# daviszhen/plan

Hardware: AMD Instinct MI355X
Metric: rows/sec through hash-agg (Q1) (higher is better)
Workload: dtype int64; 1 GPU; TPC-H Q1 fused filter+hash-aggregate over lineitem, 59986052 rows on rank 0, 59986052 in total (SF10 per GPU), table resident in HBM; rows_per_gpu=59986052, kernel_family=lowcard_chain, groups=4, rows_aggregated=58682142, parallelism=single GPU, rccl_ranks=1

## Files before the change

### include/planhip.h

```cpp
#ifndef PLANHIP_H
#define PLANHIP_H

#include <stdint.h>

#ifdef __cplusplus
extern "C" {
#endif

#define PH_OK 0
#define PH_EINVAL (-1)
#define PH_EHIP (-2)
#define PH_EUNSUPPORTED (-3)
#define PH_EOVERFLOW (-4)
#define PH_ECAPACITY (-5)
#define PH_ECONSTRAINT (-6)

typedef struct ph_ctx ph_ctx;

const char *ph_last_error(void);
const char *ph_version(void);

int ph_ctx_create(int device, ph_ctx **out);
int ph_ctx_set_stream(ph_ctx *ctx, void *hip_stream);
int ph_ctx_sync(ph_ctx *ctx);
// ... 153 lines not shown

#define PH_STAT_ASCENDING 1
#define PH_STAT_STRICT 2
#define PH_STAT_DECLARED_UNIQUE 4
int ph_table_col_stats(const ph_table *t, int32_t c, int32_t *flags);
int32_t ph_table_col_run_len(const ph_table *t, int32_t c);
int ph_table_col_narrow(const ph_table *t, int32_t c, int32_t *width, int64_t *base);
int64_t ph_table_narrow_bytes(const ph_table *t);
int ph_table_declare_unique(ph_table *t, int32_t ncols, const int32_t *cols);
int ph_table_colocate(ph_table *t, int32_t ncols, const int32_t *cols);
int32_t ph_table_colocated(const ph_table *t, int32_t ncols, const int32_t *cols);
int ph_table_set_colocate_budget(ph_table *t, int64_t bytes);
int64_t ph_table_colocate_bytes(const ph_table *t);
int ph_table_pack_scan_group(ph_table *t, int32_t ncols, const int32_t *cols);
int64_t ph_table_scan_group_bytes(const ph_table *t);
int ph_pack_scan_layout(int32_t nfields, const int32_t *widths, int32_t *shifts);
int32_t ph_pack_scan_bits(uint64_t span);
void ph_table_free(ph_table *t);

int ph_dev_alloc(ph_ctx *ctx, int64_t bytes, void **dev);
int ph_dev_free(ph_ctx *ctx, void *dev);
int ph_dev_free_many(ph_ctx *ctx, void *const *devs, int64_t n);
int ph_dev_upload(ph_ctx *ctx, void *dev, const void *host, int64_t bytes);
int ph_dev_download(ph_ctx *ctx, void *host, const void *dev, int64_t bytes);
int ph_dev_memset(ph_ctx *ctx, void *dev, int value, int64_t bytes);

typedef enum { PH_EQ = 1, PH_NE, PH_LT, PH_LE, PH_GT, PH_GE, PH_LIKE, PH_NOTLIKE } ph_cmp;

typedef struct {
    int32_t type;
// ... 347 lines not shown
```

### plan_amd/csrc/common.h

```cpp
#pragma once

#include <hip/hip_runtime.h>

#include <atomic>
#include <cstdarg>
#include <cstdint>
#include <cstdio>
#include <cstdlib>
#include <cstring>
#include <deque>
#include <map>
#include <mutex>
#include <string>
#include <vector>

#include "dispatch.h"
#include "planhip.h"

namespace ph {

void set_error(const char *fmt, ...);

#define PH_HIP(call)                                                                     \
    do {                                                                                 \
// ... 132 lines not shown
        void *data = nullptr;
        int64_t bytes = 0;
        void *ready = nullptr;
        hipStream_t built_on = nullptr;
        bool complete = false;
    };
    std::deque<colgroup> groups;
    std::map<std::vector<int>, int> sparse_gathers;
    bool replicated = false;
    int64_t colocate_budget = 4ll << 30;
    int64_t colocate_bytes = 0;
    struct scangroup {
        std::vector<int> cols;
        int32_t shift[6] = {0, 0, 0, 0, 0, 0}, width[6] = {0, 0, 0, 0, 0, 0};
        int32_t nk1 = 0, nslots = 0;
        void *data = nullptr;
        int64_t bytes = 0;
        void *ready = nullptr;
        hipStream_t built_on = nullptr;
        bool complete = false;
    };
    std::deque<scangroup> scan_groups;
    std::map<std::vector<int>, int64_t> lean_rows;
    int64_t scan_group_bytes = 0;
};

namespace ph {
template <auto Kernel>
int raise_lds(ph_ctx *ctx, int bytes) {
    static std::atomic<int> raised[64];
// ... 2 lines not shown
    int current = -1;
    PH_HIP(hipGetDevice(&current));
    if (current != ctx->device) {
        ph::set_error("raise_lds: the current device is %d, the context's is %d", current, ctx->device);
        return PH_EINVAL;
    }
    PH_HIP(hipFuncSetAttribute(reinterpret_cast<const void *>(Kernel), hipFuncAttributeMaxDynamicSharedMemorySize, bytes));
    r.store(bytes, std::memory_order_release);
    return PH_OK;
}

void register_table(ph_table *t);
void unregister_table(ph_table *t);
bool lookup_table_col(const void *data, ph_table **t, int *col);
int colocated_group_for(ph_ctx *ctx, ph_table *t, const std::vector<int> &tc, bool may_build, bool explicit_request, ph_table::colgroup *out);
int scan_group_for(ph_ctx *ctx, ph_table *t, const int32_t cols[7], int64_t rows, bool explicit_request, ph_table::scangroup *out);
bool scan_pack_enabled();
int table_finish_column(ph_ctx *ctx, ph_table::column &d, int64_t nrows, int64_t padded, const void *dict_blob, int64_t dict_bytes);
bool narrow_enabled();
}

constexpr int64_t PH_ROW_PAD = 8192;
```

### plan_amd/csrc/ctx.hip

```cpp
#include <algorithm>

#include "common.h"
#include "scan_kernels.h"

namespace ph {

static thread_local char g_err[512] = "";

void set_error(const char *fmt, ...) {
    va_list ap;
    va_start(ap, fmt);
    vsnprintf(g_err, sizeof g_err, fmt, ap);
    va_end(ap);
}

}

extern "C" const char *ph_last_error(void) { return ph::g_err; }
extern "C" const char *ph_version(void) { return "planhip 0.1 (gfx950)"; }

int ph_ctx::ensure_scratch(int64_t bytes) {
    if (bytes <= scratch_bytes) return PH_OK;
    if (scratch) {
        PH_HIP(hipStreamSynchronize(stream));
// ... 857 lines not shown
    int shift[ph::PACK_NFIELDS];
};
__global__ __launch_bounds__(256) void pack_scan_kernel(PackScanParams P, int64_t n, unsigned long long *__restrict__ out) {
    for (int64_t r = (int64_t)blockIdx.x * 256 + threadIdx.x; r < n; r += (int64_t)gridDim.x * 256) {
        unsigned long long word = (unsigned long long)((unsigned)P.k0[r] * (unsigned)P.nk1 + (unsigned)P.k1[r]) << P.shift[ph::PF_SLOT];
        for (int c = 0; c < 5; c++) {
            const unsigned long long code = P.w[c] == 1   ? ((const uint8_t *)P.src[c])[r]
                                            : P.w[c] == 2 ? ((const uint16_t *)P.src[c])[r]
                                                          : ((const uint32_t *)P.src[c])[r];
            word |= code << P.shift[c];
        }
        out[r] = word;
    }
}

namespace ph {
bool scan_pack_enabled() {
    static const bool on = !(getenv("PH_SCAN_PACK") && getenv("PH_SCAN_PACK")[0] == '0');
    return on;
}
}

static int64_t scan_pack_min_bytes() {
    if (const char *e = getenv("PH_SCAN_PACK_MIN_BYTES")) return atoll(e);
    return 256ll << 20;
}

static bool scan_group_shape(const ph_table *t, const int32_t cols[7], ph_table::scangroup *g, std::string *why) {
    auto no = [&](const std::string &s) { *why = s; return false; };
    if (!ph::narrow_enabled()) return no("the narrowed copies are switched off");
    for (int i = 0; i < 7; i++) {
        if (cols[i] < 0 || cols[i] >= (int32_t)t->cols.size()) return no("bad column " + std::to_string(cols[i]));
        for (int j = 0; j < i; j++) if (cols[j] == cols[i]) return no("column " + std::to_string(cols[i]) + " is named twice");
    }
    static const int want_w[5] = {2, 1, 4, 1, 1};
    int32_t width[ph::PACK_NFIELDS];
    for (int i = 0; i < 5; i++) {
        const ph_table::column &c = t->cols[(size_t)cols[i]];
        const bool i32 = c.type == PH_I32 || c.type == PH_DATE, i64 = c.type == PH_I64 || c.type == PH_DEC64;
        if (c.validity || !(i < 2 ? i32 : i64)) return no("column " + std::to_string(cols[i]) + " is NULL-able or not of its role's integer type");
// ... 7 lines not shown
        n[i] = c.dict.empty() ? (int)c.max + 1 : (int)c.dict.size();
        if (!c.has_range || c.min < 0 || c.max >= n[i]) return no("column " + std::to_string(cols[5 + i]) + " holds codes outside its dictionary");
    }
    if (n[0] * n[1] <= 0 || n[0] * n[1] > ph::LC_MAX_SLOTS) return no(std::to_string(n[0] * n[1]) + " group slots exceed " + std::to_string(ph::LC_MAX_SLOTS));
    g->nk1 = n[1];
    g->nslots = n[0] * n[1];
    width[ph::PF_SLOT] = ph::pack_bits((uint64_t)(g->nslots - 1));
    if (!ph::pack_layout(ph::PACK_NFIELDS, width, g->shift)) return no("the fields do not fit one 64-bit word without straddling its dwords");
    g->cols.assign(cols, cols + 7);
    std::copy(width, width + ph::PACK_NFIELDS, g->width);
    return true;
}

static int pack_scan_locked(ph_ctx *ctx, ph_table *t, ph_table::scangroup g, bool explicit_request) {
    const int64_t padded = ph::round_up(t->nrows > 0 ? t->nrows : 1, PH_ROW_PAD);
    g.bytes = padded * 8;
    if (!explicit_request && t->colocate_bytes + t->scan_group_bytes + g.bytes > t->colocate_budget) return PH_ECAPACITY;
    PH_HIP(hipSetDevice(ctx->device));
    PH_HIP(hipMalloc(&g.data, (size_t)g.bytes));
    hipEvent_t ev = nullptr;
    if (hipEventCreateWithFlags(&ev, hipEventDisableTiming) != hipSuccess) { (void)hipFree(g.data); ph::set_error("ph_table_pack_scan_group: hipEventCreate failed"); return PH_EHIP; }
    auto fail = [&]() { (void)hipEventDestroy(ev); (void)hipFree(g.data); ph::set_error("ph_table_pack_scan_group: launch failed"); return PH_EHIP; };
    if (hipMemsetAsync((char *)g.data + t->nrows * 8, 0, (size_t)((padded - t->nrows) * 8), ctx->stream) != hipSuccess) return fail();
    if (t->nrows > 0) {
        PackScanParams P{};
        for (int i = 0; i < 5; i++) { P.src[i] = t->cols[(size_t)g.cols[(size_t)i]].narrow; P.w[i] = t->cols[(size_t)g.cols[(size_t)i]].narrow_w; }
        P.k0 = (const uint8_t *)t->cols[(size_t)g.cols[5]].data;
        P.k1 = (const uint8_t *)t->cols[(size_t)g.cols[6]].data;
        P.nk1 = g.nk1;
        for (int f = 0; f < ph::PACK_NFIELDS; f++) P.shift[f] = g.shift[f];
        pack_scan_kernel<<<(int)std::min<int64_t>((t->nrows + 255) / 256, 256 * 16), 256, 0, ctx->stream>>>(P, t->nrows, (unsigned long long *)g.data);
        if (hipGetLastError() != hipSuccess) return fail();
    }
    if (hipEventRecord(ev, ctx->stream) != hipSuccess) return fail();
    g.ready = ev;
    g.built_on = ctx->stream;
    t->scan_group_bytes += g.bytes;
    t->scan_groups.push_back(g);
    return PH_OK;
}

int ph::scan_group_for(ph_ctx *ctx, ph_table *t, const int32_t cols[7], int64_t rows, bool explicit_request, ph_table::scangroup *out) {
    if (!explicit_request && !scan_pack_enabled()) return PH_EUNSUPPORTED;
    std::lock_guard<std::mutex> lock(t->mu);
    const std::vector<int> key(cols, cols + 7);
    auto find = [&]() -> ph_table::scangroup * {
        for (auto &g : t->scan_groups) if (g.cols == key) return &g;
        return nullptr;
    };
    ph_table::scangroup *g = find();
    if (!g) {
        if (explicit_request) {
            ph_table::scangroup shape;
            std::string why;
            if (!scan_group_shape(t, cols, &shape, &why)) { ph::set_error("ph_table_pack_scan_group: %s", why.c_str()); return PH_EUNSUPPORTED; }
            PH_CHECK(pack_scan_locked(ctx, t, shape, true));
        } else {
            int64_t &seen = t->lean_rows[key];
            if (seen < 0) return PH_EUNSUPPORTED;
            seen += rows;
            if (seen < 2 * t->nrows || t->nrows <= 0) return PH_EUNSUPPORTED;
            const int64_t padded = ph::round_up(t->nrows, PH_ROW_PAD);
            if (padded * 11 <= scan_pack_min_bytes()) { seen = 2 * t->nrows; return PH_EUNSUPPORTED; }
            ph_table::scangroup shape;
            std::string why;
            if (!scan_group_shape(t, cols, &shape, &why) || pack_scan_locked(ctx, t, shape, false) != PH_OK) {
                (void)hipGetLastError();
                seen = -1;
                return PH_EUNSUPPORTED;
            }
        }
        g = find();
        if (!g) return PH_EUNSUPPORTED;
    }
    if (!g->complete && g->built_on != ctx->stream) {
        const hipError_t q = hipEventQuery((hipEvent_t)g->ready);
        if (q == hipSuccess) g->complete = true;
        else if (q == hipErrorNotReady) PH_HIP(hipStreamWaitEvent(ctx->stream, (hipEvent_t)g->ready, 0));
        else { ph::set_error("packed scan group: %s", hipGetErrorString(q)); return PH_EHIP; }
    }
    *out = *g;
    return PH_OK;
}

extern "C" int ph_table_pack_scan_group(ph_table *t, int32_t ncols, const int32_t *cols) {
    PH_REQUIRE(t && t->ctx && cols && ncols == 7, "ph_table_pack_scan_group: seven columns (predicate, q, e, d, t and the two group columns)");
    ph_table::scangroup g;
    return ph::scan_group_for(t->ctx, t, cols, 0, true, &g);
}

extern "C" int64_t ph_table_scan_group_bytes(const ph_table *t) {
    if (!t) return -1;
    std::lock_guard<std::mutex> lock(const_cast<ph_table *>(t)->mu);
    return t->scan_group_bytes;
}

extern "C" int ph_pack_scan_layout(int32_t nfields, const int32_t *widths, int32_t *shifts) {
    PH_REQUIRE(widths && shifts, "ph_pack_scan_layout: bad arguments");
    if (!ph::pack_layout(nfields, widths, shifts)) { ph::set_error("ph_pack_scan_layout: the fields do not fit one 64-bit word without straddling its dwords"); return PH_EUNSUPPORTED; }
    return PH_OK;
}

extern "C" int32_t ph_pack_scan_bits(uint64_t span) { return ph::pack_bits(span); }
// ... 47 lines not shown
```

### plan_amd/csrc/pack_layout.h

```cpp
#pragma once
#include <cstdint>

namespace ph {

constexpr int PACK_NFIELDS = 6;
enum PackField { PF_P = 0, PF_Q, PF_E, PF_D, PF_T, PF_SLOT };

constexpr int pack_bits(uint64_t span) {
    int b = 1;
    while (b < 64 && (span >> b) != 0) b++;
    return b;
}

constexpr bool pack_layout(int n, const int32_t *width, int32_t *shift) {
    if (n < 1 || n > 64) return false;
    bool placed[64] = {};
    int used[2] = {0, 0};
    for (int i = 0; i < n; i++)
        if (width[i] < 1 || width[i] > 32) return false;
    for (int k = 0; k < n; k++) {
        int best = -1;
        for (int i = 0; i < n; i++)
            if (!placed[i] && (best < 0 || width[i] > width[best])) best = i;
        const int dw = used[0] + width[best] <= 32 ? 0 : used[1] + width[best] <= 32 ? 1 : -1;
// ... 5 lines not shown
    return true;
}

struct PackLayout {
    int32_t width[PACK_NFIELDS], shift[PACK_NFIELDS];
    bool ok;
};
constexpr PackLayout lineitem_pack_layout() {
    PackLayout L = {{12, 6, 24, 4, 4, 3}, {}, false};
    L.ok = pack_layout(PACK_NFIELDS, L.width, L.shift);
    return L;
}
constexpr PackLayout LCP_LINEITEM = lineitem_pack_layout();
static_assert(LCP_LINEITEM.ok, "lineitem's 53 bits fit one word");

inline bool is_lineitem_layout(const uint8_t *shift, const uint8_t *width) {
    for (int f = 0; f < PACK_NFIELDS; f++)
        if (shift[f] != LCP_LINEITEM.shift[f] || width[f] != LCP_LINEITEM.width[f]) return false;
    return true;
}

}
```

### plan_amd/csrc/scan_inst.h

```cpp
#pragma once
#include <algorithm>
#include <cstdint>

namespace ph {

enum ScanForm : int32_t { FORM_WIDE = 0, FORM_NARROW = 1, FORM_NARROW32 = 2 };

constexpr int LC_BINS_MAX_SLOTS = 6;
constexpr int LC_BINS_MAX_TILES = 1023;

struct ScanSwitches {
    bool nt = true, narrow_generic = false, pack_generic = false, lean = true, tail = true, hist = true;
    int unroll = 1, grid = 0;
};

enum FsInst { FSI_WIDE, FSI_NARROW_RT64, FSI_NARROW_RT32, FSI_NARROW_FIXED32 };
enum LcInst { LCI_WIDE, LCI_NARROW_RT64, LCI_NARROW_RT32, LCI_NARROW_FIXED32, LCI_LEAN, LCI_PACKED_RT, LCI_PACKED_FIXED, LCI_BINS };

inline FsInst narrow_inst(int32_t form, bool lineitem_widths, const ScanSwitches &s) {
    if (form == FORM_NARROW) return FSI_NARROW_RT64;
    return !s.nt || s.narrow_generic || !lineitem_widths ? FSI_NARROW_RT32 : FSI_NARROW_FIXED32;
}

struct FsFacts {
    int32_t form = FORM_WIDE;
    int32_t w[4] = {0, 0, 0, 0};
};
inline FsInst fs_choose(const FsFacts &f, const ScanSwitches &s) {
    if (f.form == FORM_WIDE) return FSI_WIDE;
    return narrow_inst(f.form, f.w[0] == 2 && f.w[1] == 1 && f.w[2] == 1 && f.w[3] == 4, s);
}
inline const char *fs_variant_name(FsInst i) {
    return i == FSI_WIDE ? "wide" : i == FSI_NARROW_RT64 ? "narrow64" : i == FSI_NARROW_RT32 ? "narrow_rt" : "narrow32";
}

struct LcFacts {
    int32_t form = FORM_WIDE;
    int32_t w[5] = {0, 0, 0, 0, 0};
    bool lean = false, group_bound = false, group_lineitem = false;
    int32_t nslots = 0;
    bool tiles_fit = true;
};
inline LcInst lc_choose(const LcFacts &f, const ScanSwitches &s) {
    if (f.group_bound) {
        const bool fixed = f.group_lineitem && !s.pack_generic;
        if (fixed && s.hist && f.nslots <= LC_BINS_MAX_SLOTS && f.tiles_fit) return LCI_BINS;
        return fixed ? LCI_PACKED_FIXED : LCI_PACKED_RT;
    }
    if (f.form == FORM_WIDE) return LCI_WIDE;
    const FsInst n = narrow_inst(f.form, f.w[0] == 2 && f.w[1] == 1 && f.w[2] == 4 && f.w[3] == 1 && f.w[4] == 1, s);
    return n == FSI_NARROW_RT64 ? LCI_NARROW_RT64 : n == FSI_NARROW_RT32 ? LCI_NARROW_RT32 : f.lean ? LCI_LEAN : LCI_NARROW_FIXED32;
}
inline bool lc_takes_lean(LcFacts f, const ScanSwitches &s) {
    f.group_bound = false;
    return lc_choose(f, s) == LCI_LEAN;
}
inline bool lc_takes_bins(LcInst i) { return i == LCI_BINS; }
inline const char *lc_variant_name(LcInst i) {
    return i == LCI_WIDE ? "wide" : i == LCI_NARROW_RT64 ? "narrow64" : i == LCI_NARROW_RT32 ? "narrow_rt" : i == LCI_NARROW_FIXED32 ? "narrow32"
         : i == LCI_LEAN ? "narrow32_lean" : "packed64";
}
inline const char *lc_row_body_name(LcInst i) { return lc_takes_bins(i) ? "bins" : "columns"; }

struct ScanGeometry {
    int64_t tile_rows, tiles;
    int grid;
    bool bins;
};
inline ScanGeometry scan_geometry(int64_t row_begin, int64_t rows, bool narrow, int max_grid, int grid_override, bool bins_eligible, int partials_cap) {
    ScanGeometry g;
    g.tile_rows = narrow ? 4096 : 1024;
    const int64_t span = rows > 0 && narrow ? rows + (row_begin & 15) : rows;
    g.tiles = (span + g.tile_rows - 1) / g.tile_rows;
    if (grid_override > 0) max_grid = std::min(grid_override, partials_cap);
    g.grid = (int)std::min<int64_t>(max_grid, std::max<int64_t>(g.tiles, 1));
    g.bins = bins_eligible;
    if (g.bins && (g.tiles + g.grid - 1) / g.grid > LC_BINS_MAX_TILES) {
        const int64_t need = (g.tiles + LC_BINS_MAX_TILES - 1) / LC_BINS_MAX_TILES;
        if (need <= partials_cap) g.grid = (int)need;
        else g.bins = false;
    }
    return g;
}

}
```

### plan_amd/csrc/scan_kernels.h

```cpp
#pragma once
#include "common.h"
#include "pack_layout.h"
#include "scan_inst.h"

namespace ph {

constexpr int LC_NACC = 6;
constexpr int LC_MAX_SLOTS = 12;
constexpr int SCAN_TAIL_MAX_ACC = 128;
struct ScanTail {
    unsigned *done;
    unsigned long long *out_lo;
    long long *out_hi;
    int32_t nacc, min_stride;
    unsigned long long *mbox;
    unsigned long long *flag;
    unsigned long long seq;
};

struct ForCol {
    const uint8_t *data;
    int64_t base;
    int32_t w;
};
// ... 20 lines not shown
    const uint8_t *k0, *k1;
    int32_t p_lo, p_hi;
    int32_t nk1;
    int32_t nslots;
    int64_t A1, B1, A2, B2;
    int64_t row_begin, row_end;
    long long *partials;
    ScanTail tail;
    int32_t form;
    ForCol np, nq, ne, nd, nt;
    uint32_t np_lo, np_hi;
    int32_t lean;
    int32_t A1c, B1c, A2c, B2c, e_base32;
    const uint8_t *pk;
    uint8_t pk_shift[PACK_NFIELDS], pk_width[PACK_NFIELDS];
    int32_t bins;
};

int launch_filter_sumprod(ph_ctx *ctx, const FilterSumProdParams &P, FsInst inst, const ScanSwitches &sw, int grid);
int launch_lowcard_chain(ph_ctx *ctx, const LowcardChainParams &P, LcInst inst, const ScanSwitches &sw, int grid);
int launch_merge_partials(ph_ctx *ctx, const long long *partials, int nblocks, int nacc,
                          int min_stride, unsigned long long *out_lo, long long *out_hi, const ScanTail *publish = nullptr);

int launch_merge_partials_ops(ph_ctx *ctx, const long long *partials, int nblocks, int nacc, int stride,
                              unsigned long long opmask, unsigned long long *out_lo, long long *out_hi, const ScanTail *publish = nullptr);

}
```

### plan_amd/csrc/scan_kernels.hip

```cpp

#include "common.h"
#include "scan_kernels.h"

namespace ph {


__device__ __forceinline__ long long wave_sum_i64(long long v) {
    for (int o = 32; o > 0; o >>= 1) v += __shfl_xor(v, o);
    return v;
}

struct alignas(16) i64x2 { long long x, y; };
struct alignas(16) i32x4 { int x, y, z, w; };

typedef long long v2i64 __attribute__((ext_vector_type(2)));
typedef int v4i32 __attribute__((ext_vector_type(4)));

template <bool NT> __device__ __forceinline__ i64x2 ld_i64x2(const int64_t *p) {
    if (NT) {
        v2i64 v = __builtin_nontemporal_load(reinterpret_cast<const v2i64 *>(p));
        return i64x2{v.x, v.y};
    }
    return *reinterpret_cast<const i64x2 *>(p);
}
// ... 809 lines not shown
    lds_char *c32 = (lds_char *)(cols + threadIdx.x);

    const int64_t tile_rows = 4096;
    const bool none = P.np_lo > P.np_hi;
    const unsigned sp = P.np_hi - P.np_lo;
    const int64_t rb = P.row_begin, re = none ? 0 : P.row_end;
    int64_t tile0 = (rb & ~(int64_t)15) + (int64_t)blockIdx.x * tile_rows;
    int64_t row = tile0 + (threadIdx.x >> 6) * (8 * LCP_GROUP) + (threadIdx.x & 63) * 2;
    const int64_t stride = (int64_t)gridDim.x * tile_rows;
#define LCH_BODY(M, T) lch_rows<M>(LCP_ARGS(T), P, row, rb, re, sp, b64, c32)
    PH_LEAN_TILE_LOOP(LCP_DECL, LCP_LOAD, LCH_BODY)
#undef LCH_BODY
    lch_fold(P, lds_acc, bins, cols, red, ns);
}

__device__ __forceinline__ void merge_finish(const ScanTail &T, int j, unsigned long long lo, long long hi, unsigned long long *out_lo, long long *out_hi) {
    const int lane = threadIdx.x;
    if (!T.done) {
        if (lane == 0) {
            out_lo[j] = lo;
            out_hi[j] = hi;
        }
        return;
    }
    unsigned ticket = 0;
    if (lane == 0) {
        __hip_atomic_store(out_lo + j, lo, __ATOMIC_RELAXED, __HIP_MEMORY_SCOPE_AGENT);
        __hip_atomic_store(out_hi + j, hi, __ATOMIC_RELAXED, __HIP_MEMORY_SCOPE_AGENT);
        __builtin_amdgcn_s_waitcnt(0);
        ticket = __hip_atomic_fetch_add(T.done, 1u, __ATOMIC_RELAXED, __HIP_MEMORY_SCOPE_AGENT);
// ... 104 lines not shown
    return PH_OK;
}

template <auto Kernel>
static int launch_lowcard_inst(ph_ctx *ctx, const LowcardChainParams &P, int grid, size_t lds) {
    PH_CHECK(raise_lds<Kernel>(ctx, 160 * 1024));
    Kernel<<<grid, 256, lds, ctx->stream>>>(P);
    PH_HIP(hipGetLastError());
    return PH_OK;
}

int launch_lowcard_chain(ph_ctx *ctx, const LowcardChainParams &P, LcInst inst, const ScanSwitches &sw, int grid) {
    const size_t lds = (size_t)P.nslots * (5 * 256 * sizeof(unsigned long long) + 2 * 256 * sizeof(unsigned));
    switch (inst) {
    case LCI_BINS: return launch_lowcard_inst<lowcard_chain_kernel_hist>(ctx, P, grid, lch_lds_bytes(P.nslots));
    case LCI_PACKED_FIXED: return launch_lowcard_inst<lowcard_chain_kernel_packed<true>>(ctx, P, grid, lds);
    case LCI_PACKED_RT: return launch_lowcard_inst<lowcard_chain_kernel_packed<false>>(ctx, P, grid, lds);
    case LCI_LEAN: return launch_lowcard_inst<lowcard_chain_kernel_lean>(ctx, P, grid, lds);
    case LCI_NARROW_FIXED32: return launch_lowcard_inst<lowcard_chain_kernel_for<true, true, 2, 1, 4, 1, 1>>(ctx, P, grid, lds);
    case LCI_NARROW_RT64: case LCI_NARROW_RT32:
        return dispatch_bool(sw.nt, [&](auto NT) { return dispatch_bool(inst == LCI_NARROW_RT32, [&](auto P32) {
            return launch_lowcard_inst<lowcard_chain_kernel_for<NT(), P32(), 0, 0, 0, 0, 0>>(ctx, P, grid, lds);
        }); });
    case LCI_WIDE:
        if (!sw.nt) return launch_lowcard_inst<lowcard_chain_kernel<false, 1>>(ctx, P, grid, lds);
        return dispatch_int<3, 2, 1>(sw.unroll, [&](auto U) { return launch_lowcard_inst<lowcard_chain_kernel<true, U()>>(ctx, P, grid, lds); });
    }
    return PH_EINVAL;
}

// ... 22 lines not shown
```

### plan_amd/csrc/scan_plan.hip

```cpp
#include <algorithm>
#include <cmath>

#include "common.h"
#include "scan_inst.h"
#include "scan_jit.h"
#include "scan_kernels.h"
#include "scan_lower.h"

namespace {

using ph::set_error;
using ph::Affine;
using ph::AggReq;
using ph::ColView;
using ph::Prod;
using ph::Range;

std::vector<ColView> col_views(const ph_table *t) {
    std::vector<ColView> v(t->cols.size());
    for (size_t i = 0; i < v.size(); i++) {
        const auto &c = t->cols[i];
        v[i] = ColView{c.type, c.scale, c.validity != nullptr, c.has_range, c.min, c.max, &c.dict};
    }
    return v;
// ... 90 lines not shown

extern "C" void ph_scan_plan_free(ph_scan_plan *p) {
    if (!p) return;
    if (p->partials) p->ctx->pool_release(p->partials);
    if (p->out_lo) p->ctx->pool_release(p->out_lo);
    if (p->g_agg) ph_agg_free(p->g_agg);
    delete p;
}


static ph::FsFacts fs_facts(const ph::FilterSumProdParams &P) { return ph::FsFacts{P.form, {P.np0.w, P.np2.w, P.nb.w, P.na.w}}; }

static ph::LcFacts lc_facts(const ph::LowcardChainParams &P, bool tiles_fit) {
    const bool group = P.pk != nullptr;
    return ph::LcFacts{P.form, {P.np.w, P.nq.w, P.ne.w, P.nd.w, P.nt.w}, P.lean != 0, group, group && ph::is_lineitem_layout(P.pk_shift, P.pk_width),
                       P.nslots, tiles_fit};
}

extern "C" const char *ph_scan_plan_kind(const ph_scan_plan *p) {
    if (!p) return "";
    return p->kind == PK_FILTER_SUMPROD ? "filter_sumprod" : p->kind == PK_LOWCARD_CHAIN ? "lowcard_chain" : p->kind == PK_JIT ? "jit" : "generic";
}

extern "C" int32_t ph_scan_plan_bytes_per_row(const ph_scan_plan *p) { return p ? p->bytes_per_row : 0; }

extern "C" const char *ph_scan_plan_variant(const ph_scan_plan *p) {
    if (!p) return "";
    if (p->kind == PK_FILTER_SUMPROD) return ph::fs_variant_name(ph::fs_choose(fs_facts(p->fs), process_switches()));
    if (p->kind == PK_LOWCARD_CHAIN) return ph::lc_variant_name(ph::lc_choose(lc_facts(p->lc, true), process_switches()));
    return ph_scan_plan_kind(p);
}

extern "C" const char *ph_scan_plan_row_body(const ph_scan_plan *p) {
    if (!p || p->kind != PK_LOWCARD_CHAIN || !(p->last_inst < 0 || p->last_inst == ph::LCI_BINS)) return "columns";
    ph::ScanSwitches sw = process_switches();
    sw.hist = hist_switch();
    return ph::lc_row_body_name(ph::lc_choose(lc_facts(p->lc, true), sw));
}


static int plan_filter_sumprod(ph_ctx *ctx, const ph_table *t, const std::vector<ColView> &cols, const std::vector<Range> &ranges,
                               const std::vector<AggReq> &reqs, ph_scan_plan *p) {
    p->kind = PK_FILTER_SUMPROD;
    int32_t a_col = -1, b_col = -1;
    for (size_t i = 0; i < reqs.size(); i++) {
        ph::AggMap m{reqs[i].kind, 1, 0};
        if (!reqs[i].star) {
            const Prod &pr = reqs[i].p;
            if (pr.f.size() != 2 || !pr.f[0].pure() || !pr.f[1].pure() || !is_i64(cols[pr.f[0].col]) || !is_i64(cols[pr.f[1].col])) {
// ... 467 lines not shown
    return sw;
}

static int bind_scan_group(ph_scan_plan *p, int64_t rows, const ph::ScanSwitches &sw) {
    if (p->lc.pk || !ph::lc_takes_lean(lc_facts(p->lc, true), sw)) return PH_OK;
    ph_table::scangroup g;
    const int rc = ph::scan_group_for(p->ctx, const_cast<ph_table *>(p->t), p->lc_cols, rows, false, &g);
    if (rc == PH_EUNSUPPORTED) return PH_OK;
    PH_CHECK(rc);
    if (g.nk1 != p->lc.nk1 || g.nslots != p->lc.nslots) return PH_OK;
    for (int f = 0; f < ph::PACK_NFIELDS; f++) {
        p->lc.pk_shift[f] = (uint8_t)g.shift[f];
        p->lc.pk_width[f] = (uint8_t)g.width[f];
    }
    p->lc.pk = (const uint8_t *)g.data;
    p->bytes_per_row = 8;
    return PH_OK;
}

static int arm_tail(ph_scan_plan *p, bool back_to_back, ph::ScanTail *tail) {
    *tail = ph::ScanTail{};
    if (!process_switches().tail || p->nacc > ph::SCAN_TAIL_MAX_ACC || (back_to_back && p->kind != PK_FILTER_SUMPROD)) return PH_OK;
    ph_ctx *ctx = p->ctx;
    if (!ctx->scan_done_dev) {
        PH_HIP(hipMalloc((void **)&ctx->scan_done_dev, 64));
        PH_HIP(hipMemsetAsync(ctx->scan_done_dev, 0, 64, ctx->stream));
    }
    tail->done = ctx->scan_done_dev;
    tail->out_lo = p->out_lo;
    tail->out_hi = p->out_hi;
    tail->nacc = p->nacc;
// ... 36 lines not shown
    PH_CHECK(ph::launch_lowcard_chain(p->ctx, P, inst, sw, grid));
    return ph::launch_merge_partials(p->ctx, p->partials, grid, p->nacc, ph::LC_NACC + 1, p->out_lo, p->out_hi, &tail);
}

extern "C" int ph_scan_plan_run(ph_scan_plan *p, int64_t row_begin, int64_t row_end) {
    PH_REQUIRE(p != nullptr, "ph_scan_plan_run: plan is NULL");
    const bool narrow = (p->kind == PK_FILTER_SUMPROD && p->fs.form != ph::FORM_WIDE) || (p->kind == PK_LOWCARD_CHAIN && p->lc.form != ph::FORM_WIDE);
    PH_REQUIRE(row_begin >= 0 && row_end >= row_begin && row_end <= p->t->nrows && (narrow || row_begin % 4 == 0),
               "ph_scan_plan_run: rows [%lld,%lld) invalid (begin must be a multiple of 4 unless the plan reads narrowed copies; table has %lld rows)",
               (long long)row_begin, (long long)row_end, (long long)p->t->nrows);
    if (p->kind == PK_GENERIC) return generic_run(p, row_begin, row_end);
    const ph::ScanSwitches sw = run_switches(p);
    const bool lowcard = p->kind == PK_LOWCARD_CHAIN;
    if (lowcard) PH_CHECK(bind_scan_group(p, row_end - row_begin, sw));
    const int64_t rows = p->never ? 0 : row_end - row_begin;
    const bool bins_eligible = lowcard && ph::lc_choose(lc_facts(p->lc, true), sw) == ph::LCI_BINS;
    const ph::ScanGeometry g = ph::scan_geometry(row_begin, rows, narrow, p->max_grid, sw.grid, bins_eligible, partials_cap(p));
    const ph::LcInst inst = lowcard ? ph::lc_choose(lc_facts(p->lc, g.bins), sw) : ph::LCI_WIDE;
    if (lowcard) p->last_inst = inst;
    const long double rows_per_block = (long double)((g.tiles + g.grid - 1) / g.grid) * (long double)g.tile_rows;
    if (p->row_bound * rows_per_block >= 4.0e18L) {
        set_error("decimal overflow proof failed: per-row bound %.3Lg x %.0Lf rows per workgroup", p->row_bound, rows_per_block);
        return PH_EOVERFLOW;
    }
    p->last_rows = rows;
    p->last_grid = g.grid;
    p->armed_seq = 0;
    const bool back_to_back = p->unfetched;
    p->unfetched = true;
    ph::ScanTail tail;
    PH_CHECK(arm_tail(p, back_to_back, &tail));
    if (p->kind == PK_FILTER_SUMPROD) return launch_filter_sumprod_plan(p, row_begin, rows, sw, g.grid, tail);
// ... 130 lines not shown
```

### plan_amd/hip.py

```python
import ctypes
import os

import numpy as np

_HERE = os.path.dirname(os.path.abspath(__file__))
_LIB = None

PH_JOIN_KEY_RANGE, PH_JOIN_FK_PROBES, PH_JOIN_KEYS_SORTED_UNIQUE, PH_JOIN_EXISTS_ONLY = 1, 2, 4, 8
PH_OK, PH_EINVAL, PH_EHIP, PH_EUNSUPPORTED, PH_EOVERFLOW, PH_ECAPACITY, PH_ECONSTRAINT = 0, -1, -2, -3, -4, -5, -6
PH_I32, PH_I64, PH_DATE, PH_DEC64, PH_CODE8, PH_F32, PH_F64, PH_STR = range(1, 9)
PH_EQ, PH_NE, PH_LT, PH_LE, PH_GT, PH_GE, PH_LIKE, PH_NOTLIKE = range(1, 9)
PH_X_COL, PH_X_CONST, PH_X_ADD, PH_X_SUB, PH_X_MUL = range(1, 6)
PH_A_SUM, PH_A_AVG, PH_A_COUNT, PH_A_MIN, PH_A_MAX, PH_A_COUNT_STAR, PH_A_COUNT_DISTINCT = range(1, 8)
PH_COMM_ID_BYTES = 128
PH_CSV_QUOTES = 1
PH_PARQUET_SNAPPY = 1
PH_PARQUET_DELTA = 4
PH_PARQUET_LZ4_RAW = 16
PH_PARQUET_GZIP = 64
PH_PARQUET_ZSTD = 256
PH_RED_SUM, PH_RED_MAX, PH_RED_MIN = 1, 2, 3

i32, i64, vp = ctypes.c_int32, ctypes.c_int64, ctypes.c_void_p

# ... 290 lines not shown
    def colocated(self, cols):
        return bool(lib().ph_table_colocated(self.h, i32(len(cols)), (i32 * len(cols))(*cols)))

    def set_replicated(self, on=True):
        check(lib().ph_table_set_replicated(self.h, i32(1 if on else 0)))

    def set_colocate_budget(self, nbytes):
        check(lib().ph_table_set_colocate_budget(self.h, i64(nbytes)))

    def colocate_bytes(self):
        lib().ph_table_colocate_bytes.restype = i64
        return int(lib().ph_table_colocate_bytes(self.h))

    def pack_scan_group(self, cols):
        check(lib().ph_table_pack_scan_group(self.h, i32(len(cols)), (i32 * len(cols))(*cols)))

    def scan_group_bytes(self):
        lib().ph_table_scan_group_bytes.restype = i64
        return int(lib().ph_table_scan_group_bytes(self.h))

    def free(self):
        if self.h:
            lib().ph_table_free(self.h)
            self.h = None


def csv_parse_field(typ, scale, field):
    field = bytes(field)
    value, null = i64(0), i32(0)
    rc = lib().ph_csv_parse_field(i32(typ), i32(scale), ctypes.c_char_p(field), i64(len(field)), ctypes.byref(value), ctypes.byref(null))
# ... 1191 lines not shown
```

Before: 725.2 billion rows/s.

## Add split56 scan-group layout packing lineitem rows into seven bytes

Adds a new packed scan-group form that stores each lineitem row in 7 bytes instead of 8. Per 1024-row block it keeps a low dword per row and packs the three 24-bit high parts of each quad into three dwords. A new pack kernel builds this layout, and new lowcard chain kernels (bins and columns variants) decode it with byte-permute instructions. The automatic path selects it for lineitem-shaped groups above a size threshold. It aims to cut HBM bytes read per row by one eighth, in exchange for extra decode ALU work and 4096-row tile anchoring.

```diff
diff --git a/include/planhip.h b/include/planhip.h
--- a/include/planhip.h
+++ b/include/planhip.h
@@ -191,6 +191,9 @@
 int64_t ph_table_colocate_bytes(const ph_table *t);
 int ph_table_pack_scan_group(ph_table *t, int32_t ncols, const int32_t *cols);
 int64_t ph_table_scan_group_bytes(const ph_table *t);
+#define PH_SCAN_GROUP_WORD64 0
+#define PH_SCAN_GROUP_SPLIT56 1
+int ph_table_pack_scan_group_ex(ph_table *t, int32_t ncols, const int32_t *cols, int32_t form);
 int ph_pack_scan_layout(int32_t nfields, const int32_t *widths, int32_t *shifts);
 int32_t ph_pack_scan_bits(uint64_t span);
 void ph_table_free(ph_table *t);
diff --git a/plan_amd/csrc/common.h b/plan_amd/csrc/common.h
--- a/plan_amd/csrc/common.h
+++ b/plan_amd/csrc/common.h
@@ -170,6 +170,7 @@
         std::vector<int> cols;
         int32_t shift[6] = {0, 0, 0, 0, 0, 0}, width[6] = {0, 0, 0, 0, 0, 0};
         int32_t nk1 = 0, nslots = 0;
+        int32_t form = 0;
         void *data = nullptr;
         int64_t bytes = 0;
         void *ready = nullptr;
@@ -202,7 +203,7 @@
 void unregister_table(ph_table *t);
 bool lookup_table_col(const void *data, ph_table **t, int *col);
 int colocated_group_for(ph_ctx *ctx, ph_table *t, const std::vector<int> &tc, bool may_build, bool explicit_request, ph_table::colgroup *out);
-int scan_group_for(ph_ctx *ctx, ph_table *t, const int32_t cols[7], int64_t rows, bool explicit_request, ph_table::scangroup *out);
+int scan_group_for(ph_ctx *ctx, ph_table *t, const int32_t cols[7], int64_t rows, bool explicit_request, ph_table::scangroup *out, int32_t form = 0);
 bool scan_pack_enabled();
 int table_finish_column(ph_ctx *ctx, ph_table::column &d, int64_t nrows, int64_t padded, const void *dict_blob, int64_t dict_bytes);
 bool narrow_enabled();
diff --git a/plan_amd/csrc/ctx.hip b/plan_amd/csrc/ctx.hip
--- a/plan_amd/csrc/ctx.hip
+++ b/plan_amd/csrc/ctx.hip
@@ -895,6 +895,30 @@
     }
 }
 
+__global__ __launch_bounds__(256) void pack_split_kernel(PackScanParams P, int64_t n, int64_t nquads, unsigned *__restrict__ out) {
+    for (int64_t q = (int64_t)blockIdx.x * 256 + threadIdx.x; q < nquads; q += (int64_t)gridDim.x * 256) {
+        unsigned lo[4], hi[4], d[3];
+        for (int k = 0; k < 4; k++) {
+            const int64_t r = q * 4 + k;
+            unsigned long long word = 0;
+            if (r < n)
+                word = (unsigned long long)((unsigned)P.k0[r] * (unsigned)P.nk1 + (unsigned)P.k1[r]) << P.shift[ph::PF_SLOT] |
+                       (unsigned long long)((const uint16_t *)P.src[ph::PF_P])[r] << P.shift[ph::PF_P] |
+                       (unsigned long long)((const uint8_t *)P.src[ph::PF_Q])[r] << P.shift[ph::PF_Q] |
+                       (unsigned long long)((const uint32_t *)P.src[ph::PF_E])[r] << P.shift[ph::PF_E] |
+                       (unsigned long long)((const uint8_t *)P.src[ph::PF_D])[r] << P.shift[ph::PF_D] |
+                       (unsigned long long)((const uint8_t *)P.src[ph::PF_T])[r] << P.shift[ph::PF_T];
+            lo[k] = (unsigned)word;
+            hi[k] = (unsigned)(word >> 32);
+        }
+        ph::split_quad_encode(hi, d);
+        const int r0 = (int)(q * 4 % ph::SPLIT_BLOCK_ROWS);
+        unsigned *block = out + q * 4 / ph::SPLIT_BLOCK_ROWS * ph::SPLIT_BLOCK_DWORDS;
+        *reinterpret_cast<uint4 *>(block + ph::split_low_dword(r0)) = make_uint4(lo[0], lo[1], lo[2], lo[3]);
+        for (int i = 0; i < 3; i++) block[ph::split_high_dword(r0, i)] = d[i];
+    }
+}
+
 namespace ph {
 bool scan_pack_enabled() {
     static const bool on = !(getenv("PH_SCAN_PACK") && getenv("PH_SCAN_PACK")[0] == '0');
@@ -905,6 +929,19 @@
 static int64_t scan_pack_min_bytes() {
     if (const char *e = getenv("PH_SCAN_PACK_MIN_BYTES")) return atoll(e);
     return 256ll << 20;
+}
+
+static int64_t scan_split_min_bytes() {
+    if (const char *e = getenv("PH_SCAN_SPLIT_MIN_BYTES")) return atoll(e);
+    return 256ll << 20;
+}
+static bool scan_split_enabled() {
+    const char *e = getenv("PH_SCAN_SPLIT");
+    return !(e && e[0] == '0');
+}
+static bool scan_pack_generic() {
+    static const bool on = getenv("PH_SCAN_PACK_GENERIC") && getenv("PH_SCAN_PACK_GENERIC")[0] == '1';
+    return on;
 }
 
 static bool scan_group_shape(const ph_table *t, const int32_t cols[7], ph_table::scangroup *g, std::string *why) {
@@ -942,14 +979,17 @@
 
 static int pack_scan_locked(ph_ctx *ctx, ph_table *t, ph_table::scangroup g, bool explicit_request) {
     const int64_t padded = ph::round_up(t->nrows > 0 ? t->nrows : 1, PH_ROW_PAD);
-    g.bytes = padded * 8;
+    static_assert(PH_ROW_PAD % 4096 == 0, "a 4096-row tile that starts inside the padded table lies inside a split group");
+    const bool split = g.form == ph::SG_SPLIT56;
+    g.bytes = split ? ph::split_group_bytes(padded) : padded * 8;
     if (!explicit_request && t->colocate_bytes + t->scan_group_bytes + g.bytes > t->colocate_budget) return PH_ECAPACITY;
     PH_HIP(hipSetDevice(ctx->device));
     PH_HIP(hipMalloc(&g.data, (size_t)g.bytes));
     hipEvent_t ev = nullptr;
     if (hipEventCreateWithFlags(&ev, hipEventDisableTiming) != hipSuccess) { (void)hipFree(g.data); ph::set_error("ph_table_pack_scan_group: hipEventCreate failed"); return PH_EHIP; }
     auto fail = [&]() { (void)hipEventDestroy(ev); (void)hipFree(g.data); ph::set_error("ph_table_pack_scan_group: launch failed"); return PH_EHIP; };
-    if (hipMemsetAsync((char *)g.data + t->nrows * 8, 0, (size_t)((padded - t->nrows) * 8), ctx->stream) != hipSuccess) return fail();
+    const int64_t filled = split ? ph::split_group_bytes(ph::round_up(t->nrows, ph::SPLIT_BLOCK_ROWS)) : t->nrows * 8;
+    if (hipMemsetAsync((char *)g.data + filled, 0, (size_t)(g.bytes - filled), ctx->stream) != hipSuccess) return fail();
     if (t->nrows > 0) {
         PackScanParams P{};
         for (int i = 0; i < 5; i++) { P.src[i] = t->cols[(size_t)g.cols[(size_t)i]].narrow; P.w[i] = t->cols[(size_t)g.cols[(size_t)i]].narrow_w; }
@@ -957,7 +997,11 @@
         P.k1 = (const uint8_t *)t->cols[(size_t)g.cols[6]].data;
         P.nk1 = g.nk1;
         for (int f = 0; f < ph::PACK_NFIELDS; f++) P.shift[f] = g.shift[f];
-        pack_scan_kernel<<<(int)std::min<int64_t>((t->nrows + 255) / 256, 256 * 16), 256, 0, ctx->stream>>>(P, t->nrows, (unsigned long long *)g.data);
+        if (split) {
+            const int64_t nquads = ph::round_up(t->nrows, ph::SPLIT_BLOCK_ROWS) / 4;
+            pack_split_kernel<<<(int)std::min<int64_t>((nquads + 255) / 256, 256 * 16), 256, 0, ctx->stream>>>(P, t->nrows, nquads, (unsigned *)g.data);
+        } else
+            pack_scan_kernel<<<(int)std::min<int64_t>((t->nrows + 255) / 256, 256 * 16), 256, 0, ctx->stream>>>(P, t->nrows, (unsigned long long *)g.data);
         if (hipGetLastError() != hipSuccess) return fail();
     }
     if (hipEventRecord(ev, ctx->stream) != hipSuccess) return fail();
@@ -968,8 +1012,10 @@
     return PH_OK;
 }
 
-int ph::scan_group_for(ph_ctx *ctx, ph_table *t, const int32_t cols[7], int64_t rows, bool explicit_request, ph_table::scangroup *out) {
+int ph::scan_group_for(ph_ctx *ctx, ph_table *t, const int32_t cols[7], int64_t rows, bool explicit_request, ph_table::scangroup *out, int32_t form) {
     if (!explicit_request && !scan_pack_enabled()) return PH_EUNSUPPORTED;
+    const bool split_on = scan_split_enabled();
+    if (explicit_request && form == ph::SG_SPLIT56 && !split_on) { ph::set_error("ph_table_pack_scan_group: the split form is switched off (PH_SCAN_SPLIT=0)"); return PH_EUNSUPPORTED; }
     std::lock_guard<std::mutex> lock(t->mu);
     const std::vector<int> key(cols, cols + 7);
     auto find = [&]() -> ph_table::scangroup * {
@@ -982,6 +1028,11 @@
             ph_table::scangroup shape;
             std::string why;
             if (!scan_group_shape(t, cols, &shape, &why)) { ph::set_error("ph_table_pack_scan_group: %s", why.c_str()); return PH_EUNSUPPORTED; }
+            if (form == ph::SG_SPLIT56 && !ph::is_lineitem_layout(shape.shift, shape.width)) {
+                ph::set_error("ph_table_pack_scan_group: the split form exists for lineitem's field layout only");
+                return PH_EUNSUPPORTED;
+            }
+            shape.form = form;
             PH_CHECK(pack_scan_locked(ctx, t, shape, true));
         } else {
             int64_t &seen = t->lean_rows[key];
@@ -992,7 +1043,10 @@
             if (padded * 11 <= scan_pack_min_bytes()) { seen = 2 * t->nrows; return PH_EUNSUPPORTED; }
             ph_table::scangroup shape;
             std::string why;
-            if (!scan_group_shape(t, cols, &shape, &why) || pack_scan_locked(ctx, t, shape, false) != PH_OK) {
+            const bool ok = scan_group_shape(t, cols, &shape, &why);
+            if (ok && split_on && !scan_pack_generic() && ph::is_lineitem_layout(shape.shift, shape.width) && padded * 8 > scan_split_min_bytes())
+                shape.form = ph::SG_SPLIT56;
+            if (!ok || pack_scan_locked(ctx, t, shape, false) != PH_OK) {
                 (void)hipGetLastError();
                 seen = -1;
                 return PH_EUNSUPPORTED;
@@ -1000,7 +1054,11 @@
         }
         g = find();
         if (!g) return PH_EUNSUPPORTED;
-    }
+    } else if (explicit_request && g->form != form) {
+        ph::set_error("ph_table_pack_scan_group: the column set already has a group of the other form (%s)", g->form == ph::SG_SPLIT56 ? "split56" : "word64");
+        return PH_EUNSUPPORTED;
+    }
+    if (g->form == ph::SG_SPLIT56 && !split_on) return PH_EUNSUPPORTED;
     if (!g->complete && g->built_on != ctx->stream) {
         const hipError_t q = hipEventQuery((hipEvent_t)g->ready);
         if (q == hipSuccess) g->complete = true;
@@ -1015,6 +1073,13 @@
     PH_REQUIRE(t && t->ctx && cols && ncols == 7, "ph_table_pack_scan_group: seven columns (predicate, q, e, d, t and the two group columns)");
     ph_table::scangroup g;
     return ph::scan_group_for(t->ctx, t, cols, 0, true, &g);
+}
+
+extern "C" int ph_table_pack_scan_group_ex(ph_table *t, int32_t ncols, const int32_t *cols, int32_t form) {
+    PH_REQUIRE(t && t->ctx && cols && ncols == 7, "ph_table_pack_scan_group_ex: seven columns (predicate, q, e, d, t and the two group columns)");
+    PH_REQUIRE(form == ph::SG_WORD64 || form == ph::SG_SPLIT56, "ph_table_pack_scan_group_ex: form %d is neither word64 (0) nor split56 (1)", (int)form);
+    ph_table::scangroup g;
+    return ph::scan_group_for(t->ctx, t, cols, 0, true, &g, form);
 }
 
 extern "C" int64_t ph_table_scan_group_bytes(const ph_table *t) {
diff --git a/plan_amd/csrc/pack_layout.h b/plan_amd/csrc/pack_layout.h
--- a/plan_amd/csrc/pack_layout.h
+++ b/plan_amd/csrc/pack_layout.h
@@ -43,10 +43,45 @@
 constexpr PackLayout LCP_LINEITEM = lineitem_pack_layout();
 static_assert(LCP_LINEITEM.ok, "lineitem's 53 bits fit one word");
 
-inline bool is_lineitem_layout(const uint8_t *shift, const uint8_t *width) {
+template <class T> inline bool is_lineitem_layout(const T *shift, const T *width) {
     for (int f = 0; f < PACK_NFIELDS; f++)
         if (shift[f] != LCP_LINEITEM.shift[f] || width[f] != LCP_LINEITEM.width[f]) return false;
     return true;
 }
 
+enum ScanGroupForm : int32_t { SG_WORD64 = 0, SG_SPLIT56 = 1 };
+
+constexpr int SPLIT_HIGH_BITS = 24;
+constexpr bool split_layout_fits(const PackLayout &L) {
+    int low = 0;
+    for (int f = 0; f < PACK_NFIELDS; f++) {
+        if (L.shift[f] >= 32 && L.shift[f] - 32 + L.width[f] > SPLIT_HIGH_BITS) return false;
+        if (L.shift[f] < 32) low += L.width[f];
+    }
+    return low <= 32;
 }
+static_assert(split_layout_fits(LCP_LINEITEM), "lineitem's high-dword fields end below bit 24 and its low-dword fields fill no more than 32 bits");
+
+constexpr int SPLIT_BLOCK_ROWS = 1024, SPLIT_LOW_DWORDS = 1024, SPLIT_BLOCK_DWORDS = 1792, SPLIT_BLOCK_BYTES = SPLIT_BLOCK_DWORDS * 4;
+constexpr int64_t split_group_bytes(int64_t padded_rows) { return padded_rows / SPLIT_BLOCK_ROWS * SPLIT_BLOCK_BYTES; }
+
+constexpr int split_lane(int r) { return (r >> 2) & 63; }
+constexpr int split_load(int r) { return r >> 8; }
+constexpr int split_role(int r) { return r & 3; }
+constexpr int split_low_dword(int r) { return r; }
+constexpr int split_lane_high_dword(int l, int i) { return SPLIT_LOW_DWORDS + 256 * (i >> 2) + 4 * l + (i & 3); }
+constexpr int split_high_dword(int r, int r3) { return split_lane_high_dword(split_lane(r), 3 * split_load(r) + r3); }
+
+constexpr void split_quad_encode(const uint32_t h[4], uint32_t d[3]) {
+    d[0] = h[0] | (h[3] & 0xffu) << 24;
+    d[1] = h[1] | (h[3] >> 8 & 0xffu) << 24;
+    d[2] = h[2] | (h[3] >> 16) << 24;
+}
+constexpr void split_quad_decode(const uint32_t d[3], uint32_t h[4]) {
+    h[0] = d[0] & 0xffffffu;
+    h[1] = d[1] & 0xffffffu;
+    h[2] = d[2] & 0xffffffu;
+    h[3] = d[0] >> 24 | d[1] >> 24 << 8 | d[2] >> 24 << 16;
+}
+
+}
diff --git a/plan_amd/csrc/scan_inst.h b/plan_amd/csrc/scan_inst.h
--- a/plan_amd/csrc/scan_inst.h
+++ b/plan_amd/csrc/scan_inst.h
@@ -15,7 +15,7 @@
 };
 
 enum FsInst { FSI_WIDE, FSI_NARROW_RT64, FSI_NARROW_RT32, FSI_NARROW_FIXED32 };
-enum LcInst { LCI_WIDE, LCI_NARROW_RT64, LCI_NARROW_RT32, LCI_NARROW_FIXED32, LCI_LEAN, LCI_PACKED_RT, LCI_PACKED_FIXED, LCI_BINS };
+enum LcInst { LCI_WIDE, LCI_NARROW_RT64, LCI_NARROW_RT32, LCI_NARROW_FIXED32, LCI_LEAN, LCI_PACKED_RT, LCI_PACKED_FIXED, LCI_BINS, LCI_SPLIT_COLUMNS, LCI_SPLIT_BINS };
 
 inline FsInst narrow_inst(int32_t form, bool lineitem_widths, const ScanSwitches &s) {
     if (form == FORM_NARROW) return FSI_NARROW_RT64;
@@ -40,11 +40,14 @@
     bool lean = false, group_bound = false, group_lineitem = false;
     int32_t nslots = 0;
     bool tiles_fit = true;
+    bool group_split = false;
 };
 inline LcInst lc_choose(const LcFacts &f, const ScanSwitches &s) {
     if (f.group_bound) {
         const bool fixed = f.group_lineitem && !s.pack_generic;
-        if (fixed && s.hist && f.nslots <= LC_BINS_MAX_SLOTS && f.tiles_fit) return LCI_BINS;
+        const bool bins = fixed && s.hist && f.nslots <= LC_BINS_MAX_SLOTS && f.tiles_fit;
+        if (f.group_split) return bins ? LCI_SPLIT_BINS : LCI_SPLIT_COLUMNS;
+        if (bins) return LCI_BINS;
         return fixed ? LCI_PACKED_FIXED : LCI_PACKED_RT;
     }
     if (f.form == FORM_WIDE) return LCI_WIDE;
@@ -55,10 +58,11 @@
     f.group_bound = false;
     return lc_choose(f, s) == LCI_LEAN;
 }
-inline bool lc_takes_bins(LcInst i) { return i == LCI_BINS; }
+inline bool lc_takes_bins(LcInst i) { return i == LCI_BINS || i == LCI_SPLIT_BINS; }
+inline bool lc_takes_split(LcInst i) { return i == LCI_SPLIT_COLUMNS || i == LCI_SPLIT_BINS; }
 inline const char *lc_variant_name(LcInst i) {
     return i == LCI_WIDE ? "wide" : i == LCI_NARROW_RT64 ? "narrow64" : i == LCI_NARROW_RT32 ? "narrow_rt" : i == LCI_NARROW_FIXED32 ? "narrow32"
-         : i == LCI_LEAN ? "narrow32_lean" : "packed64";
+         : i == LCI_LEAN ? "narrow32_lean" : lc_takes_split(i) ? "split56" : "packed64";
 }
 inline const char *lc_row_body_name(LcInst i) { return lc_takes_bins(i) ? "bins" : "columns"; }
 
@@ -67,10 +71,11 @@
     int grid;
     bool bins;
 };
-inline ScanGeometry scan_geometry(int64_t row_begin, int64_t rows, bool narrow, int max_grid, int grid_override, bool bins_eligible, int partials_cap) {
+inline ScanGeometry scan_geometry(int64_t row_begin, int64_t rows, bool narrow, int max_grid, int grid_override, bool bins_eligible, int partials_cap,
+                                   int64_t anchor = 16) {
     ScanGeometry g;
     g.tile_rows = narrow ? 4096 : 1024;
-    const int64_t span = rows > 0 && narrow ? rows + (row_begin & 15) : rows;
+    const int64_t span = rows > 0 && narrow ? rows + (row_begin & (anchor - 1)) : rows;
     g.tiles = (span + g.tile_rows - 1) / g.tile_rows;
     if (grid_override > 0) max_grid = std::min(grid_override, partials_cap);
     g.grid = (int)std::min<int64_t>(max_grid, std::max<int64_t>(g.tiles, 1));
diff --git a/plan_amd/csrc/scan_kernels.h b/plan_amd/csrc/scan_kernels.h
--- a/plan_amd/csrc/scan_kernels.h
+++ b/plan_amd/csrc/scan_kernels.h
@@ -58,7 +58,8 @@
     int32_t A1c, B1c, A2c, B2c, e_base32;
     const uint8_t *pk;
     uint8_t pk_shift[PACK_NFIELDS], pk_width[PACK_NFIELDS];
-    int32_t bins;
+    int16_t bins;
+    int16_t pk_form;
 };
 
 int launch_filter_sumprod(ph_ctx *ctx, const FilterSumProdParams &P, FsInst inst, const ScanSwitches &sw, int grid);
diff --git a/plan_amd/csrc/scan_kernels.hip b/plan_amd/csrc/scan_kernels.hip
--- a/plan_amd/csrc/scan_kernels.hip
+++ b/plan_amd/csrc/scan_kernels.hip
@@ -847,6 +847,87 @@
     lch_fold(P, lds_acc, bins, cols, red, ns);
 }
 
+#define LCS_DECL(T) v4u32 T##l0, T##l1, T##l2, T##l3, T##h0, T##h1, T##h2
+#define LCS_ARGS(T) T##l0, T##l1, T##l2, T##l3, T##h0, T##h1, T##h2
+#define LCS_LOAD(T, R, T0)                                                                       \
+    do {                                                                                         \
+        (void)row_safe;                \
+        const int64_t t_ = (T0) < re ? (T0) : tile_first;                                        \
+        const uint8_t *b_ = lane_base + t_ * (SPLIT_BLOCK_BYTES / SPLIT_BLOCK_ROWS);             \
+        T##l0 = ld_u32x4<true>(b_);                                                              \
+        T##l1 = ld_u32x4<true>(b_ + 1024);                                                       \
+        T##l2 = ld_u32x4<true>(b_ + 2048);                                                       \
+        T##l3 = ld_u32x4<true>(b_ + 3072);                                                       \
+        T##h0 = ld_u32x4<true>(b_ + 4096);                                                       \
+        T##h1 = ld_u32x4<true>(b_ + 5120);                                                       \
+        T##h2 = ld_u32x4<true>(b_ + 6144);                                                       \
+    } while (0)
+static_assert(SPLIT_BLOCK_BYTES % SPLIT_BLOCK_ROWS == 0 && SPLIT_BLOCK_BYTES == 7 * 1024 && SPLIT_LOW_DWORDS * 4 == 4096,
+              "a block is seven loads of 1024 bytes per wave, the high parts from byte 4096 on");
+
+__device__ __forceinline__ unsigned lcs_row3(unsigned A, unsigned B, unsigned C) {
+    const unsigned ab = __builtin_amdgcn_perm(B, A, 0x0c0c0703u);
+    return __builtin_amdgcn_perm(C, ab, 0x0c070100u);
+}
+
+template <bool MASKED, bool BINS>
+__device__ __forceinline__ void lcs_rows(const v4u32 l0, const v4u32 l1, const v4u32 l2, const v4u32 l3, const v4u32 h0, const v4u32 h1, const v4u32 h2,
+                                         const LowcardChainParams &P, int64_t row, int64_t rb, int64_t re, unsigned sp, lds_char *la, lds_char *lb) {
+    int a1c = P.A1c, a2c = P.A2c;
+    if constexpr (!BINS) asm volatile("" : "+v"(a1c), "+v"(a2c));
+    auto one = [&](unsigned lo, unsigned hi, int64_t r) {
+        if constexpr (BINS) lch_row<MASKED>(P, lo, hi, r, rb, re, sp, la, lb);
+        else lcp_row<MASKED, true>(P, lo, hi, r, rb, re, sp, la, lb, a1c, a2c);
+    };
+#define LCS_QUAD(L, A, B, C, J)                          \
+    one(L.x, A, row + 256 * (J));                        \
+    one(L.y, B, row + 256 * (J) + 1);                    \
+    one(L.z, C, row + 256 * (J) + 2);                    \
+    one(L.w, lcs_row3(A, B, C), row + 256 * (J) + 3)
+    LCS_QUAD(l0, h0.x, h0.y, h0.z, 0);
+    LCS_QUAD(l1, h0.w, h1.x, h1.y, 1);
+    LCS_QUAD(l2, h1.z, h1.w, h2.x, 2);
+    LCS_QUAD(l3, h2.y, h2.z, h2.w, 3);
+#undef LCS_QUAD
+}
+
+template <bool BINS> __global__ __launch_bounds__(256, 2) void lowcard_chain_kernel_split(LowcardChainParams P) {
+    extern __shared__ __attribute__((aligned(16))) unsigned long long lds_acc[];
+    const int ns = P.nslots;
+    unsigned long long *bins = lds_acc, *red = lds_acc + (size_t)5 * ns * 256, *lds64 = lds_acc;
+    unsigned *cols = reinterpret_cast<unsigned *>(lds_acc + (size_t)4 * ns * 256), *lds32 = reinterpret_cast<unsigned *>(lds_acc + (size_t)ns * 5 * 256);
+    lds_char *la, *lb;
+    if constexpr (BINS) {
+        for (int i = threadIdx.x; i < 4 * ns * 256; i += 256) bins[i] = 0;
+        for (int s = 0; s < ns; s++) {
+            cols[(s * 2 + 0) * 256 + threadIdx.x] = 0;
+            cols[(s * 2 + 1) * 256 + threadIdx.x] = 0xffffffffu;
+        }
+        __syncthreads();
+        la = (lds_char *)(bins + (size_t)(threadIdx.x >> 6) * ns * 256);
+        lb = (lds_char *)(cols + threadIdx.x);
+    } else {
+        lc_lds_init(lds64, lds32, ns);
+        la = (lds_char *)(lds64 + threadIdx.x);
+        lb = (lds_char *)(lds32 + threadIdx.x);
+    }
+
+    const int64_t tile_rows = 4096;
+    const bool none = P.np_lo > P.np_hi;
+    const unsigned sp = P.np_hi - P.np_lo;
+    const int64_t rb = P.row_begin, re = none ? 0 : P.row_end;
+    const int64_t tile_first = rb & ~(tile_rows - 1);
+    int64_t tile0 = tile_first + (int64_t)blockIdx.x * tile_rows;
+    int64_t row = tile0 + (threadIdx.x >> 6) * SPLIT_BLOCK_ROWS + (threadIdx.x & 63) * 4;
+    const uint8_t *lane_base = P.pk + (threadIdx.x >> 6) * SPLIT_BLOCK_BYTES + (threadIdx.x & 63) * 16;
+    const int64_t stride = (int64_t)gridDim.x * tile_rows;
+#define LCS_BODY(M, T) lcs_rows<M, BINS>(LCS_ARGS(T), P, row, rb, re, sp, la, lb)
+    PH_LEAN_TILE_LOOP(LCS_DECL, LCS_LOAD, LCS_BODY)
+#undef LCS_BODY
+    if constexpr (BINS) lch_fold(P, lds_acc, bins, cols, red, ns);
+    else lc_merge(P, lds_acc, lds64, lds32, ns);
+}
+
 __device__ __forceinline__ void merge_finish(const ScanTail &T, int j, unsigned long long lo, long long hi, unsigned long long *out_lo, long long *out_hi) {
     const int lane = threadIdx.x;
     if (!T.done) {
@@ -981,6 +1062,8 @@
     const size_t lds = (size_t)P.nslots * (5 * 256 * sizeof(unsigned long long) + 2 * 256 * sizeof(unsigned));
     switch (inst) {
     case LCI_BINS: return launch_lowcard_inst<lowcard_chain_kernel_hist>(ctx, P, grid, lch_lds_bytes(P.nslots));
+    case LCI_SPLIT_BINS: return launch_lowcard_inst<lowcard_chain_kernel_split<true>>(ctx, P, grid, lch_lds_bytes(P.nslots));
+    case LCI_SPLIT_COLUMNS: return launch_lowcard_inst<lowcard_chain_kernel_split<false>>(ctx, P, grid, lds);
     case LCI_PACKED_FIXED: return launch_lowcard_inst<lowcard_chain_kernel_packed<true>>(ctx, P, grid, lds);
     case LCI_PACKED_RT: return launch_lowcard_inst<lowcard_chain_kernel_packed<false>>(ctx, P, grid, lds);
     case LCI_LEAN: return launch_lowcard_inst<lowcard_chain_kernel_lean>(ctx, P, grid, lds);
diff --git a/plan_amd/csrc/scan_plan.hip b/plan_amd/csrc/scan_plan.hip
--- a/plan_amd/csrc/scan_plan.hip
+++ b/plan_amd/csrc/scan_plan.hip
@@ -128,7 +128,7 @@
 static ph::LcFacts lc_facts(const ph::LowcardChainParams &P, bool tiles_fit) {
     const bool group = P.pk != nullptr;
     return ph::LcFacts{P.form, {P.np.w, P.nq.w, P.ne.w, P.nd.w, P.nt.w}, P.lean != 0, group, group && ph::is_lineitem_layout(P.pk_shift, P.pk_width),
-                       P.nslots, tiles_fit};
+                       P.nslots, tiles_fit, group && P.pk_form == ph::SG_SPLIT56};
 }
 
 extern "C" const char *ph_scan_plan_kind(const ph_scan_plan *p) {
@@ -146,7 +146,7 @@
 }
 
 extern "C" const char *ph_scan_plan_row_body(const ph_scan_plan *p) {
-    if (!p || p->kind != PK_LOWCARD_CHAIN || !(p->last_inst < 0 || p->last_inst == ph::LCI_BINS)) return "columns";
+    if (!p || p->kind != PK_LOWCARD_CHAIN || !(p->last_inst < 0 || ph::lc_takes_bins((ph::LcInst)p->last_inst))) return "columns";
     ph::ScanSwitches sw = process_switches();
     sw.hist = hist_switch();
     return ph::lc_row_body_name(ph::lc_choose(lc_facts(p->lc, true), sw));
@@ -644,7 +644,8 @@
         p->lc.pk_width[f] = (uint8_t)g.width[f];
     }
     p->lc.pk = (const uint8_t *)g.data;
-    p->bytes_per_row = 8;
+    p->lc.pk_form = (int16_t)g.form;
+    p->bytes_per_row = g.form == ph::SG_SPLIT56 ? 7 : 8;
     return PH_OK;
 }
 
@@ -711,8 +712,9 @@
     const bool lowcard = p->kind == PK_LOWCARD_CHAIN;
     if (lowcard) PH_CHECK(bind_scan_group(p, row_end - row_begin, sw));
     const int64_t rows = p->never ? 0 : row_end - row_begin;
-    const bool bins_eligible = lowcard && ph::lc_choose(lc_facts(p->lc, true), sw) == ph::LCI_BINS;
-    const ph::ScanGeometry g = ph::scan_geometry(row_begin, rows, narrow, p->max_grid, sw.grid, bins_eligible, partials_cap(p));
+    const bool bins_eligible = lowcard && ph::lc_takes_bins(ph::lc_choose(lc_facts(p->lc, true), sw));
+    const int64_t anchor = lowcard && p->lc.pk && p->lc.pk_form == ph::SG_SPLIT56 ? 4096 : 16;
+    const ph::ScanGeometry g = ph::scan_geometry(row_begin, rows, narrow, p->max_grid, sw.grid, bins_eligible, partials_cap(p), anchor);
     const ph::LcInst inst = lowcard ? ph::lc_choose(lc_facts(p->lc, g.bins), sw) : ph::LCI_WIDE;
     if (lowcard) p->last_inst = inst;
     const long double rows_per_block = (long double)((g.tiles + g.grid - 1) / g.grid) * (long double)g.tile_rows;
diff --git a/plan_amd/hip.py b/plan_amd/hip.py
--- a/plan_amd/hip.py
+++ b/plan_amd/hip.py
@@ -328,6 +328,9 @@
 
     def pack_scan_group(self, cols):
         check(lib().ph_table_pack_scan_group(self.h, i32(len(cols)), (i32 * len(cols))(*cols)))
+
+    def pack_scan_group_ex(self, cols, form):
+        check(lib().ph_table_pack_scan_group_ex(self.h, i32(len(cols)), (i32 * len(cols))(*cols), i32(form)))
 
     def scan_group_bytes(self):
         lib().ph_table_scan_group_bytes.restype = i64
```

Result: faster. 809.5 billion rows/s (median of 6 runs) (+11.6%).
